# piljoong-jeong/nerf_meets_mlx

Measured on AMD Instinct MI355X. Metric: train+render rays/sec on Lego 800x800 (synthetic), coarse+fine 64+128, higher is better.
Workload: dtype split16 (fp16x2 render / bf16x2 train MFMA operands ~ 22 / 16 significand bits; fp32 accumulate)

## Files before the change

nerf_meets_mlx_amd/csrc/mlp.hip:

```cpp
#include "common.h"
#include "mlp_ring.h"
#include "mlp_layout.h"
#include "mlp_frag.h"
#include "mlp_arch2.h"
#include "hash_common.h"
#include "mlp_params.h"
#include "mlp_model.h"
#include "dw_split.h"
#include <limits.h>
#include <string.h>


namespace nerf {

extern int g_hash_combine_max_res;




constexpr int PACK_THREADS = (L::F_TOTAL + L::B_PADDED) * 64 + L::BI_TOTAL;
__device__ __forceinline__ void pack_part(int tid, const float* __restrict__ p, bf16x8* __restrict__ wf,
                                          bf16x8* __restrict__ wb, float* __restrict__ bias) {
  const int nf = L::F_TOTAL * 64, nb = L::B_PADDED * 64;
  if (tid < nf + nb) {
// ... 936 lines not shown
  for (int i = 0; i < DW_NPW; ++i) {
    const int nt = wr * DW_NPW + i;
    if (nt >= n_tiles) continue;
#pragma unroll
    for (int k = 0; k < 2; ++k) {
      const int kt = wc * 2 + k;
      if (kt >= k_tiles) continue;
      float* tile = slot + (8 * nt + kt) * 1024;
#pragma unroll
      for (int e = 0; e < 16; ++e) tile[((e & 3) + 8 * (e >> 2) + 4 * hh) * 32 + rr] = acc[i][k][e];
    }
    if (wc == 0 && jb.b_off >= 0) {
      const float tot = bsum[i] + __shfl_xor(bsum[i], 32, 64);
      if (hh == 0) slot[64 * 1024 + 32 * nt + rr] = tot;
    }
  }
}

__global__ void __launch_bounds__(256) mlp_dw_reduce_kernel(DwArgs a) {
  const int j = blockIdx.y;
  const DwJob jb = a.jobs[j];
  int first = 0;
  for (int q = 0; q < j; ++q) first += a.splits[q];
  const int S = a.splits[j];
  const int nw = jb.n_valid * jb.k_valid, nb = jb.b_off >= 0 ? jb.n_valid : 0;
  const float* base = a.partial + (size_t)first * DW_SLOT_FLOATS;
  for (int t = blockIdx.x * 256 + threadIdx.x; t < nw + nb; t += gridDim.x * 256) {
    const float* src;
    float* dst;
    if (t < nw) {
      const int n = t / jb.k_valid, k = t - n * jb.k_valid;
      src = base + (8 * (n >> 5) + (k >> 5)) * 1024 + (n & 31) * 32 + (k & 31);
      dst = a.grads + jb.w_off + (int64_t)n * jb.ldw + jb.col0 + k;
    } else {
      src = base + 64 * 1024 + (t - nw);
      dst = a.grads + jb.b_off + (t - nw);
    }
    float sum = 0.0f;
    int sidx = 0;
    for (; sidx + 8 <= S; sidx += 8) {
      float v[8];
#pragma unroll
      for (int q = 0; q < 8; ++q) v[q] = __builtin_nontemporal_load(src + (size_t)(sidx + q) * DW_SLOT_FLOATS);
#pragma unroll
      for (int q = 0; q < 8; ++q) sum += v[q];
    }
    for (; sidx < S; ++sidx) sum += __builtin_nontemporal_load(src + (size_t)sidx * DW_SLOT_FLOATS);
    *dst = sum;
  }
}



__global__ void __launch_bounds__(256) pack_img_kernel(const float* __restrict__ p, bf16x8* __restrict__ wf,
                                                       bf16x8* __restrict__ wb, float* __restrict__ bias, int out_ch) {
  const int tid = blockIdx.x * 256 + threadIdx.x;
  const int nf = LI::F_TOTAL * 64, nb = LI::B_PADDED * 64;
  if (tid < nf + nb) {
    const bool fw = tid < nf;
    const int t = fw ? tid : tid - nf;
    const int f = t >> 6, lane = t & 63, r = lane & 31, h = lane >> 5;
    bf16x8 v;
#pragma unroll
    for (int j = 0; j < 8; ++j)
      v[j] = (__bf16)(fw ? fwd_src_img(p, f, r, h, j, out_ch) : (f < LI::B_TOTAL ? bwd_src_img(p, f, r, h, j, out_ch) : 0.0f));
    (fw ? wf : wb)[t] = v;
  } else if (tid < nf + nb + LI::BI_TOTAL) {
    const int s = tid - nf - nb;
    bias[s] = s < 2048 ? p[LI::pb(s >> 8) + (s & 255)] : ((s - LI::BI_OUT) < out_ch ? p[LI::P_WO + out_ch * 256 + (s - LI::BI_OUT)] : 0.0f);
// ... 333 lines not shown
    {
      bf16x8 cat[ST][5];
#pragma unroll
      for (int k = 0; k < 4; ++k) cat[0][k] = zf[0][k];
      cat[0][4] = zal[0][0];
      layer_bwd<ST, 5, 2, true>(ws, LN::B_FA, cat, z1, mk[1], lane, ZSINK(LN::Z_L1));
    }
    layer_bwd<ST, 4, 2, true>(ws, LN::B_L1, z1, z0, mk[0], lane, ZSINK(LN::Z_L0));
#undef ZSINK
    if (a.d_x) {
      f32x16 acc;
#pragma unroll
      for (int i = 0; i < 16; ++i) acc[i] = 0.0f;
#pragma unroll
      for (int ns = 0; ns < 4; ++ns) acc = __builtin_amdgcn_mfma_f32_32x32x16_bf16(ws.frag(LN::B_L0 + ns, lane), z0[0][ns], acc, 0, 0, 0);
      if (m < a.M) {
#pragma unroll
        for (int q = 0; q < 4; ++q) {
          float4 o; o.x = acc[4 * q]; o.y = acc[4 * q + 1]; o.z = acc[4 * q + 2]; o.w = acc[4 * q + 3];
          *reinterpret_cast<float4*>(a.d_x + m * LN::CPOS + 8 * q + 4 * h) = o;
        }
      }
    }
  }
}

static int g_dw_wgs = 0;
static int g_dw_bias = -1;
static int g_bwd_stage = 0;
static int g_dw_ring_cap = 8;
static int g_dw_private = 4;
static int g_dw16_variant = 1;
static int g_dw_narrow_first = 1;
static int g_dw_job_mask = 0;
static int g_mlp_variant = 0;
static int g_ring_wgs = 0;
static int g_ngp_ray_major = 1;
int g_pass_queue = 1;
static int g_ring_split = 1;

static int cu_count() {
  constexpr int MAX_DEVICES = 64;
  static int n[MAX_DEVICES] = {};
  int dev = 0;
  if (hipGetDevice(&dev) != hipSuccess || dev < 0 || dev >= MAX_DEVICES) dev = 0;
  if (n[dev] == 0) {
    int v = 0;
    n[dev] = (hipDeviceGetAttribute(&v, hipDeviceAttributeMultiprocessorCount, dev) == hipSuccess && v > 0) ? v : 256;
  }
  return n[dev];
}
static inline int ring_wgs() { return g_ring_wgs > 0 ? g_ring_wgs : cu_count(); }
static inline unsigned ring_grid(int64_t ntiles) { return persistent_grid((ntiles + 7) / 8, ring_wgs()); }

struct Option { const char* key; int* var; bool (*rule)(int& v); const char* refusal; };
static bool opt_any(int&) { return true; }
static bool opt_flag(int& v) { v = v ? 1 : 0; return true; }
template <int LO, int HI> static bool opt_clamp(int& v) { v = v < LO ? LO : v > HI ? HI : v; return true; }
static const Option OPTIONS[] = {
    {"mlp_variant", &g_mlp_variant, opt_any, nullptr},
    {"ring_split", &g_ring_split, [](int& v) { return v == 1 || v == 2; }, "nerf_set_option: ring_split must be 1 or 2"},
    {"ring_workgroups", &g_ring_wgs, opt_clamp<0, INT_MAX>, nullptr},
    {"tile_pad16", &g_tile_pad16, opt_clamp<0, INT_MAX>, nullptr},
    {"dw_workgroups", &g_dw_wgs, opt_clamp<0, INT_MAX>, nullptr},
    {"dw_unit_bias", &g_dw_bias, opt_clamp<-1, INT_MAX>, nullptr},
    {"bwd_stage", &g_bwd_stage, opt_any, nullptr},
    {"dw_job_mask", &g_dw_job_mask, opt_any, nullptr},
    {"hash_combine_max_res", &g_hash_combine_max_res, opt_clamp<0, INT_MAX>, nullptr},
    {"ngp_ray_major", &g_ngp_ray_major, opt_flag, nullptr},
    {"dw22_variant", &s16::g_dw_variant, opt_flag, nullptr},
    {"dw16_variant", &g_dw16_variant, opt_clamp<0, 3>, nullptr},
    {"dw_private_tiles", &g_dw_private, opt_clamp<0, 4>, nullptr},
    {"dw_ring_cap", &g_dw_ring_cap, opt_clamp<2, 16>, nullptr},
    {"pass_queue", &g_pass_queue, opt_flag, nullptr},
    {"dw_narrow_first", &g_dw_narrow_first, opt_flag, nullptr},
    {"f22_tiles", &f22::g_tiles, [](int& v) { return v == 0 || v == 2 || v == 3; }, "nerf_set_option: f22_tiles must be 0 (automatic), 2 or 3"},
};

}

using namespace nerf;

extern "C" int nerf_set_option(const char* key, int value) {
  NERF_REQUIRE(key, NERF_E_NULL, "nerf_set_option: key is NULL");
  NERF_REQUIRE(strcmp(key, "mlp_precision") != 0, NERF_E_UNSUPPORTED,
               "nerf_set_option: \"mlp_precision\" is gone (ABI 3): set nerf_mlp_arch.precision of the model instead");
  for (const Option& o : OPTIONS) {
    if (strcmp(key, o.key)) continue;
    if (!o.rule(value)) return fail(NERF_E_UNSUPPORTED, "%s", o.refusal);
    *o.var = value;
    return NERF_OK;
  }
  return fail(NERF_E_UNSUPPORTED, "nerf_set_option: unknown key '%s'", key);
}

extern "C" int nerf_get_option(const char* key) {
  if (!key) return NERF_OPTION_UNKNOWN;
  for (const Option& o : OPTIONS)
    if (!strcmp(key, o.key)) return *o.var;
  return NERF_OPTION_UNKNOWN;
}

extern "C" int64_t nerf_mlp_param_count(const nerf_mlp_arch* arch) { return resolve(arch).params; }
extern "C" int64_t nerf_mlp_packed_bytes(const nerf_mlp_arch* arch) { return resolve(arch).packed_bytes; }
extern "C" int64_t nerf_mlp_acts_bytes(const nerf_mlp_arch* arch, int64_t M) { return resolve(arch).acts_bytes(M); }
extern "C" int64_t nerf_mlp_dz_bytes(const nerf_mlp_arch* arch, int64_t M) { return resolve(arch).dz_bytes(M); }

#define NERF_ARCH_MSG ": HIP kernels exist for (8x256, skip 4) with in=63+27 view head, or in=40 / no view head / out_ch<=4, and for (2x64, no skip) with in=32+16 view head"
// ... 130 lines not shown
}

static int view_forward(const Model& m, const void* packed, const float* x, const float* rays, const float* z, int64_t M, int n,
                        int freq_mode, float* out, void* acts, void* stream) {
  auto s = as_stream(stream);
  if (m.split() && !acts)
    return f22::forward(m.stream<void>(packed, S_F22), x, rays, z, M, n, freq_mode, out, ring_wgs(), s);
  if (m.split())
    return s16::forward(m.stream<void>(packed, S_S16), m.stream<float>(packed, S_BIAS), x, rays, z, M, n, freq_mode, out, acts,
                        m.astride(), ring_wgs(), s);
  if (m.prec == Prec::F32) return f32::forward(m.stream<void>(packed, S_F32), x, rays, z, M, n, freq_mode, out, acts, 0, s);
  return x ? launch_fwd<0>(m, packed, x, rays, z, M, n, freq_mode, out, acts, stream)
           : launch_fwd<1>(m, packed, x, rays, z, M, n, freq_mode, out, acts, stream);
}

extern "C" int nerf_mlp_forward(const nerf_mlp_arch* arch, const void* packed, const float* x, int64_t M, float* out,
                                void* stream) {
  return nerf_mlp_forward_train(arch, packed, x, M, out, nullptr, stream);
}

extern "C" int nerf_query_fused(const nerf_mlp_arch* arch, const void* packed, const float* rays, const float* z,
                                int64_t B, int n, int freq_mode, float* raw, void* acts, void* stream) {
  const Model m = resolve(arch);
  NERF_REQUIRE(m.ok && m.shape == Shape::View, NERF_E_UNSUPPORTED, "nerf_query_fused" NERF_ARCH_MSG);
  NERF_REQUIRE(n >= 1, NERF_E_SHAPE, "nerf_query_fused: n must be >= 1");
  if (B <= 0) return NERF_OK;
  NERF_REQUIRE(packed && rays && z && raw, NERF_E_NULL, "nerf_query_fused: NULL pointer");
  NERF_REQUIRE(freq_mode == 0 || freq_mode == 1, NERF_E_UNSUPPORTED, "nerf_query_fused: freq_mode must be 0 or 1");
  NERF_REQUIRE(B * (int64_t)n < (1ll << 31), NERF_E_SHAPE, "nerf_query_fused: B*n must be < 2^31 samples per call");
  return view_forward(m, packed, nullptr, rays, z, B * n, n, freq_mode, raw, acts, stream);
}

static int launch_dw_part(const Model& m, DwArgs& d, int nj, int64_t ntiles, const void* acts, void* dz, float* grads,
                          hipStream_t s, int kind, int slot_base, int max_wgs) {
  static_assert(DW_SPLIT_MAX_JOBS == DW_MAX_JOBS, "dw_split.h sizes its arrays for DwArgs::jobs");
  DwCost cost[DW_MAX_JOBS];
  for (int j = 0; j < nj; ++j) cost[j] = DwCost{d.jobs[j].nf, d.jobs[j].kf};
  int target_wgs = g_dw_wgs > 0 ? g_dw_wgs : cu_count();
  if (target_wgs > max_wgs) target_wgs = max_wgs;
  const int nw = dw_split(cost, nj, g_dw_bias >= 0 ? g_dw_bias : m.split() ? 2 : 128, target_wgs, (ntiles + 3) / 4, d.splits);
  NERF_REQUIRE(slot_base + nw <= DW_MAX_WGS, NERF_E_SHAPE, "nerf_mlp_backward: dw_workgroups must be <= %d", DW_MAX_WGS);
  bool all_tiny = true;
  for (int j = 0; j < nj; ++j) all_tiny = all_tiny && ((d.jobs[j].nf + 1) / 2) * ((d.jobs[j].kf + 1) / 2) <= 4;
  d.ntiles = (int)ntiles; d.astride = m.astride(); d.zstride = m.zstride();
  d.acts = acts; d.dz = dz; d.grads = grads;
  d.a_lo = m.info->a_lo; d.z_lo = m.info->z_lo; d.ring_cap = g_dw_ring_cap; d.private_max_tiles = g_dw_private;
  d.partial = m.dw_partial(dz, ntiles) + (size_t)slot_base * DW_SLOT_FLOATS;
  int rc;
  if (kind >= 2) {
    rc = launch_dw_wide_kernel(d, nw, kind == 2, s);
  } else if (kind == 1) {
    rc = s16::launch_dw_kernel(d, nw, true, s);
  } else if (g_dw16_variant == 3 || (g_dw16_variant == 1 && all_tiny)) {
    rc = s16::launch_dw_kernel(d, nw, false, s);
  } else {
    rc = launch<mlp_dw_kernel>("mlp dW", dim3(nw), dim3(64 * DW_WAVES), DW_LDS_BYTES, s, d);
  }
  if (rc) return rc;
  return launch<mlp_dw_reduce_kernel>("mlp dW reduce", dim3(257, nj), dim3(256), 0, s, d);
}

static int launch_dw(const Model& m, DwArgs& d, int nj, int64_t ntiles, const void* acts, void* dz, float* grads, hipStream_t s) {
  if (g_dw_job_mask) {
    hipError_t e = hipMemsetAsync(grads, 0, sizeof(float) * m.params, s);
    if (e != hipSuccess) return fail(NERF_E_HIP, "nerf_mlp_backward: memset: %s", hipGetErrorString(e));
  }
  const bool split_bf16 = m.split();
  if ((split_bf16 ? s16::g_dw_variant : g_dw16_variant) == 0)
    return launch_dw_part(m, d, nj, ntiles, acts, dz, grads, s, split_bf16 ? 1 : 0, 0, DW_MAX_WGS);
  DwArgs wide = d, rest = d;
  int nwide = 0, nrest = 0;
  for (int j = 0; j < nj; ++j) {
    if (d.jobs[j].nf == 16 && d.jobs[j].kf == 16) wide.jobs[nwide++] = d.jobs[j];
    else rest.jobs[nrest++] = d.jobs[j];
  }
  const int half = DW_MAX_WGS / 2;
  for (int turn = 0; turn < 2; ++turn) {
    const bool do_wide = (turn == 0) != (g_dw_narrow_first != 0);
    if (do_wide && nwide) {
      const int rc = launch_dw_part(m, wide, nwide, ntiles, acts, dz, grads, s, split_bf16 ? 2 : 3, half, half);
      if (rc) return rc;
    }
    if (!do_wide && nrest) {
      const int rc = launch_dw_part(m, rest, nrest, ntiles, acts, dz, grads, s, split_bf16 ? 1 : 0, 0, half);
      if (rc) return rc;
    }
  }
  return NERF_OK;
}

static int view_backward_chain(const Model& m, const void* packed, const void* acts, const float* d_raw, int64_t M, void* dz,
                               hipStream_t s) {
  const int64_t ntiles = (M + 31) / 32;
  if (m.split()) {
    if (g_bwd_stage != 2) {
      const int rcs = s16::backward_chain(m.stream<void>(packed, S_S16), acts, d_raw, M, dz, m.astride(), m.zstride(), ring_wgs(), s);
      if (rcs) return rcs;
    }
    return check_launch("mlp backward chain");
  }
  BwdArgs b;
  b.queue = nullptr;
  b.wb = m.stream<bf16x8>(packed, S_BWD);
  b.acts = acts; b.d_raw = d_raw; b.M = M; b.dz = dz; b.astride = m.astride(); b.zstride = m.zstride();
  const int variant = g_mlp_variant == 0 ? 3 : g_mlp_variant;
  const char* what = "mlp backward chain";
  if (variant >= 3) {
    b.queue = passq_slot();
    if (g_bwd_stage == 2) return check_launch(what);
    if (g_ring_split == 2)
      return launch<mlp_bwd_ring_kernel<SPLIT_NW, SPLIT_CHUNK>>(
          what, dim3(persistent_grid((ntiles + SPLIT_NW - 1) / SPLIT_NW, 2 * (int64_t)ring_wgs())), dim3(64 * SPLIT_NW), SPLIT_LDS_BYTES, s, b);
    return launch<mlp_bwd_ring_kernel<>>(what, dim3(ring_grid(ntiles)), dim3(512), RING_LDS_BYTES, s, b);
  }
  const int st = variant == 2 ? 2 : 1;
  const int64_t blocks = (ntiles + 4 * st - 1) / (4 * st);
  return with_bool(st == 1, [&](auto one) {
// ... 7 lines not shown
  NERF_REQUIRE(!d_x || m.shape == Shape::Small, NERF_E_UNSUPPORTED,
               "nerf_mlp_backward_inputs: input gradients exist for the (2x64) model only (the 8x256 models take fixed encodings)");
  NERF_REQUIRE(packed && acts && d_raw && dz && grads, NERF_E_NULL, "nerf_mlp_backward: NULL pointer");
  NERF_REQUIRE(M > 0, NERF_E_SHAPE, "nerf_mlp_backward: M must be > 0");
  auto s = as_stream(stream);
  const int64_t ntiles = (M + 31) / 32;
  if (m.prec == Prec::F32)
    return f32::backward(m.stream<void>(packed, S_F32), acts, d_raw, M, dz, grads, m.shape == Shape::Image ? m.out_ch : 0, s);
  int rc;
  if (m.shape == Shape::Small) {
    if (m.split()) {
      rc = s16x::small_backward_chain(m.stream<void>(packed, S_S16), acts, d_raw, M, dz, d_x, m.astride(), m.zstride(), s);
    } else {
      SmallArgs a;
      small_args(a, m, packed);
      a.d_raw = d_raw; a.acts = const_cast<void*>(acts); a.dz = dz; a.M = M; a.d_x = d_x;
      rc = launch<mlp_small_bwd_kernel>("mlp backward chain (2x64 model)", dim3(small_grid(ntiles)), dim3(512), LN::LDS_BYTES, s, a);
    }
  } else if (m.shape == Shape::Image) {
    if (m.split()) {
      rc = s16x::img_backward_chain(m.stream<void>(packed, S_S16), acts, d_raw, M, m.out_ch, dz, m.astride(), m.zstride(), ring_wgs(), s);
    } else {
      ImgArgs a;
      img_args(a, m, packed);
      a.d_out = d_raw; a.acts = const_cast<void*>(acts); a.dz = dz; a.M = M;
      rc = launch<mlp_img_bwd_ring_kernel>("mlp backward chain (image model)", dim3(ring_grid(ntiles)), dim3(512), RING_LDS_BYTES, s, a);
    }
  } else {
    rc = view_backward_chain(m, packed, acts, d_raw, M, dz, s);
    if (!rc && g_bwd_stage == 1) return NERF_OK;
  }
  if (rc) return rc;
  DwArgs d;
  const int nj = m.dw_jobs(d.jobs, m.shape == Shape::View ? g_dw_job_mask : 0);
  return launch_dw(m, d, nj, ntiles, acts, dz, grads, s);
}

static int ngp_query_fused_impl(const nerf_mlp_arch* arch, const void* packed, const float* rays, const float* z,
                                int64_t B, int n, const float* tables, const void* tables_half, int L, int log2_T, int F,
                                const int* resolutions_host, const float* lw_host, int sh_degree, float pos_scale,
                                float pos_offset, float* raw, void* acts, void* stream) {
  const Model m = resolve(arch);
  NERF_REQUIRE(m.ok && m.shape == Shape::Small, NERF_E_UNSUPPORTED, "nerf_ngp_query_fused: needs the (2x64, in 32+16) model");
  NERF_REQUIRE(L == 16 && F == 2 && sh_degree == 3, NERF_E_UNSUPPORTED,
               "nerf_ngp_query_fused: fused rows exist for 16 levels x 2 features + SH degree 3 (use nerf_ngp_encode + nerf_mlp_forward otherwise)");
  NERF_REQUIRE(log2_T >= 1 && log2_T <= 30, NERF_E_SHAPE, "nerf_ngp_query_fused: need 1<=log2_T<=30");
  if (B <= 0 || n <= 0) return NERF_OK;
  NERF_REQUIRE(packed && rays && z && tables && resolutions_host && raw, NERF_E_NULL, "nerf_ngp_query_fused: NULL pointer");
  const int64_t M = B * n;
  NERF_REQUIRE(M < (1ll << 31), NERF_E_SHAPE, "nerf_ngp_query_fused: B*n must be < 2^31");
  LevelTab lt;
  if (lw_host)
    NERF_REQUIRE(level_tab_fill(lt, lw_host, L), NERF_E_SHAPE, "nerf_ngp_query_fused_lw: level weights must be finite and in [0, 1]");
  if (m.split()) {
    s16x::SmallQuery q;
    q.rays = rays; q.z = z; q.n = n; q.tables = tables; q.T = 1u << log2_T; q.pos_scale = pos_scale; q.pos_offset = pos_offset;
    for (int l = 0; l < 32; ++l) q.res[l] = l < L ? (float)resolutions_host[l] : 0.0f;
    q.B = B; q.ray_major = g_ngp_ray_major;
    q.use_lw = lw_host != nullptr;
    if (lw_host) for (int l = 0; l < 32; ++l) q.lw[l] = lt.w[l];
    return s16x::small_forward(m.stream<void>(packed, S_S16), m.stream<float>(packed, S_BIAS), nullptr, M, raw, acts, m.astride(), &q,
                               as_stream(stream));
  }
  SmallArgs a;
  small_args(a, m, packed);
  a.out = raw; a.acts = acts; a.M = M; a.rays = rays; a.z = z; a.n = n; a.tables = tables; a.T = 1u << log2_T;
  a.tables_h = static_cast<const uint32_t*>(tables_half);
  a.pos_scale = pos_scale; a.pos_offset = pos_offset;
// ... 98 lines not shown
```

nerf_meets_mlx_amd/csrc/mlp_frag.h:

```cpp
#pragma once
#include "mlp_layout.h"

namespace nerf {

struct Chan { int kind, dim, band; };
__host__ __device__ constexpr Chan chan_of(int c, int limit) {
  if (c < 3) return Chan{0, c, 0};
  if (c >= limit) return Chan{3, 0, 0};
  return Chan{((c - 3) % 6) >= 3 ? 2 : 1, (c - 3) % 3, (c - 3) / 6};
}

__device__ inline float fwd_src(const float* __restrict__ p, int f, int r, int h, int j) {
  int nt, ks;
  if (f < L::F_L1) {
    nt = f / 4; ks = f % 4;
    const int kk = kperm(ks, h, j);
    return kk < 63 ? p[L::P_W0 + (32 * nt + r) * 63 + kk] : 0.0f;
  }
  if (f < L::F_L5) {
    const int l = 1 + (f - L::F_L1) / 128, g = (f - L::F_L1) % 128;
    nt = g / 16; ks = g % 16;
    return p[L::pw(l) + (32 * nt + r) * 256 + kperm(ks, h, j)];
  }
  if (f < L::F_L6) {
    const int g = f - L::F_L5;
    nt = g / 20; ks = g % 20;
    const int kk = kperm(ks, h, j), n = 32 * nt + r;
    if (kk < 64) return kk < 63 ? p[L::P_W5 + n * 319 + kk] : 0.0f;
    return p[L::P_W5 + n * 319 + 63 + (kk - 64)];
  }
  if (f < L::F_FA) {
    const int l = 6 + (f - L::F_L6) / 128, g = (f - L::F_L6) % 128;
    nt = g / 16; ks = g % 16;
    return p[L::pw(l) + (32 * nt + r) * 256 + kperm(ks, h, j)];
  }
  if (f < L::F_DIR) {
    const int g = f - L::F_FA;
    nt = g / 16; ks = g % 16;
    const int kk = kperm(ks, h, j);
    if (nt < 8) return p[L::P_WF + (32 * nt + r) * 256 + kk];
    return r == 0 ? p[L::P_WA + kk] : 0.0f;
  }
  if (f < L::F_RGB) {
    const int g = f - L::F_DIR;
    nt = g / 18; ks = g % 18;
    const int kk = kperm(ks, h, j), n = 32 * nt + r;
    if (kk < 256) return p[L::P_WD + n * 283 + kk];
    return (kk - 256) < 27 ? p[L::P_WD + n * 283 + kk] : 0.0f;
  }
  ks = f - L::F_RGB;
  return r < 3 ? p[L::P_WR + r * 128 + kperm(ks, h, j)] : 0.0f;
}

__device__ inline float bwd_src(const float* __restrict__ p, int f, int r, int h, int j) {
  if (f < L::B_DIR) {
    const int nn = kperm(0, h, j);
    return nn < 3 ? p[L::P_WR + nn * 128 + 32 * f + r] : 0.0f;
  }
  if (f < L::B_FA) {
    const int g = f - L::B_DIR, kt = g / 8, ns = g % 8;
    return p[L::P_WD + kperm(ns, h, j) * 283 + 32 * kt + r];
  }
  if (f < L::B_L7) {
    const int g = f - L::B_FA, kt = g / 17, ns = g % 17;
    const int nn = kperm(ns, h, j);
    if (ns < 16) return p[L::P_WF + nn * 256 + 32 * kt + r];
    return nn == 256 ? p[L::P_WA + 32 * kt + r] : 0.0f;
  }
  const int g = f - L::B_L7, li = g / 128, q = g % 128, kt = q / 16, ns = q % 16;
  const int l = 7 - li, nn = kperm(ns, h, j), row = 32 * kt + r;
  if (l == 5) return p[L::P_W5 + nn * 319 + 63 + row];
  return p[L::pw(l) + nn * 256 + row];
}

__device__ __forceinline__ bf16x8* frag_ptr(void* base, int64_t tile, int64_t stride16, int slot, int r, int h) {
  char* tb = reinterpret_cast<char*>(base) + tile * stride16 * 16;
  return reinterpret_cast<bf16x8*>(tb + slot * 1024 + (unsigned)(32 * r + 16 * h));
}

#ifndef NERF_NT_STORES
#define NERF_NT_STORES 1
#endif
constexpr bool g_nt_stores = NERF_NT_STORES != 0;

__device__ __forceinline__ void store_frag(void* base, int64_t tile, int64_t stride16, int slot, const bf16x8& v,
                                           int r, int h) {
#if NERF_ABLATE == 7
  asm volatile("" :: "v"(v));
  return;
#endif
#if NERF_ABLATE == 8
  tile = tile & 7;
#endif
  if (g_nt_stores) __builtin_nontemporal_store(v, frag_ptr(base, tile, stride16, slot, r, h));
  else *frag_ptr(base, tile, stride16, slot, r, h) = v;
}
template <int COUNT>
__device__ __forceinline__ void store_frags(void* base, int64_t tile, int64_t stride16, int slot0,
                                            const bf16x8 (&frags)[COUNT], int r, int h) {
#pragma unroll
  for (int k = 0; k < COUNT; ++k) store_frag(base, tile, stride16, slot0 + k, frags[k], r, h);
}
struct NoSink {
  __device__ __forceinline__ void put(int, int, const bf16x8&) const {}
};
// ... 60 lines not shown
}
template <int B>
__device__ __forceinline__ bf16x2 keep_where(bf16x2 p, unsigned w) {
  unsigned sel, r;
  asm("v_pk_lshrrev_b16 %0, %2, %1 op_sel_hi:[0,1]" : "=v"(sel) : "v"(w), "n"(B));
  sel &= 0x00010001u;
  asm("v_pk_mul_lo_u16 %0, %1, %2" : "=v"(r) : "v"(__builtin_bit_cast(unsigned, p)), "v"(sel));
  return __builtin_bit_cast(bf16x2, r);
}

template <bool RELU, bool MASKOUT>
__device__ __forceinline__ void finish_quarter(const f32x16& acc, int q, int nt, bf16x8& lo, bf16x8& hi, u32x4& mask) {
  unsigned w = 0;
#pragma unroll
  for (int p = 0; p < 2; ++p) {
    const int i = 4 * q + 2 * p, k = 2 * q + p;
    const bf16x2 pr = RELU ? relu_pack(acc[i], acc[i + 1]) : pack2(acc[i], acc[i + 1]);
    if (MASKOUT) w |= nonzero_bits(pr) << k;
    if (i < 8) { lo[i] = pr[0]; lo[i + 1] = pr[1]; } else { hi[i - 8] = pr[0]; hi[i - 7] = pr[1]; }
  }
  if (MASKOUT) mask[nt >> 1] |= w << (8 * (nt & 1));
}

__host__ __device__ constexpr int quarter_pos(int ks_count, int q) {
  return ks_count >= 8 ? (q * ks_count) / 4 + 1 : (q < ks_count ? q : ks_count - 1);
}

struct DwJob {
  int dz_slot, nf;
  int act_slot, kf;
  int w_off, ldw, col0;
  int n_valid, k_valid;
  int b_off;
};
constexpr int DW_MAX_JOBS = 16;
struct DwArgs {
  DwJob jobs[DW_MAX_JOBS];
  int splits[DW_MAX_JOBS];
  int ntiles;
  int64_t astride, zstride;
  const void* acts;
  const void* dz;
  float* grads;
  float* partial;
  int ring_cap;
  int private_max_tiles;
  int a_lo, z_lo;
};
constexpr int DW_SLOT_FLOATS = 64 * 1024 + 256;
constexpr int DW_MAX_WGS = 512;
constexpr int64_t DW_PARTIAL_BYTES = (int64_t)DW_MAX_WGS * DW_SLOT_FLOATS * 4;
int launch_dw_wide_kernel(const DwArgs& d, int workgroups, bool split_bf16, hipStream_t s);

}
```

nerf_meets_mlx_amd/csrc/mlp_layout.h:

```cpp
#pragma once
#include "mlp_ring.h"
#include "mlp_params.h"

namespace nerf {

namespace L {

constexpr int F_L0 = 0, F_L1 = 32, F_L5 = 544, F_L6 = 704, F_L7 = 832, F_FA = 960, F_DIR = 1104, F_RGB = 1176;
constexpr int F_TOTAL = 1184;
constexpr int B_RGB = 0, B_DIR = 4, B_FA = 68, B_L7 = 204, B_L6 = 332, B_L5 = 460, B_L4 = 588;
constexpr int B_TOTAL = 1100, B_PADDED = 1120;
constexpr int BI_FEAT = 2048, BI_ALPHA = 2304, BI_DIR = 2336, BI_RGB = 2464, BI_TOTAL = 2496;
constexpr int F16_TOTAL = 1172, F16_PADDED = 1184;
constexpr int64_t F16_OFFSET = (int64_t)(F_TOTAL + B_PADDED) * 1024 + BI_TOTAL * 4;
constexpr int64_t PACKED_BYTES = F16_OFFSET + (int64_t)F16_PADDED * 1024;

constexpr int A_PE = 0, A_DPE = 4, A_H0 = 6;
constexpr int A_FEAT = 134, A_HD = 150;
constexpr int A_MASK = 158, A_SLOTS = 167;
constexpr int Z_L0 = 0;
constexpr int Z_F = 128, Z_A = 144, Z_D = 145, Z_RGB = 153, Z_SLOTS = 154;
}

__host__ __device__ constexpr int kperm(int ks, int h, int j) { return 16 * ks + 8 * (j >> 2) + 4 * h + (j & 3); }

namespace L16 {
constexpr int F_L0 = 0, F_L1 = 32, F_L5 = 544, F_L6 = 704, F_L7 = 832, F_FA = 960, F_DIR = 1096, F_RGB = 1168;
constexpr int CHUNKS = L::F16_PADDED / RING_CHUNK;
}
__host__ __device__ constexpr int kperm16(int ks, int g, int j) { return 32 * ks + 16 * (j >> 2) + 4 * g + (j & 3); }
__host__ __device__ constexpr int pos_chan16(int ks, int g, int j) {
  const int sl = 8 * ks + j;
  if (sl < 12) return 3 + 6 * (2 * g + sl / 6) + (sl % 6);
  if (sl < 15) return 3 + 6 * (8 + (g >> 1)) + 3 * (g & 1) + (sl - 12);
  return g < 3 ? g : -1;
}
__host__ __device__ constexpr int dir_chan16(int g, int j) {
  if (j < 6) return 3 + 6 * g + j;
  return (j == 6 && g < 3) ? g : -1;
}

__device__ inline float fwd_src16(const float* __restrict__ p, int f, int i, int g, int j) {
  if (f < L16::F_L1) {
    const int nt = f / 2, ch = pos_chan16(f % 2, g, j);
    return ch >= 0 ? p[L::P_W0 + (16 * nt + i) * 63 + ch] : 0.0f;
  }
  if (f < L16::F_L5) {
    const int q = f - L16::F_L1, l = 1 + q / 128, r = q % 128;
    return p[L::pw(l) + (16 * (r / 8) + i) * 256 + kperm16(r % 8, g, j)];
  }
  if (f < L16::F_L6) {
    const int q = f - L16::F_L5, n = 16 * (q / 10) + i, ks = q % 10;
    if (ks < 2) { const int ch = pos_chan16(ks, g, j); return ch >= 0 ? p[L::P_W5 + n * 319 + ch] : 0.0f; }
    return p[L::P_W5 + n * 319 + 63 + kperm16(ks - 2, g, j)];
  }
  if (f < L16::F_FA) {
    const int q = f - L16::F_L6, l = 6 + q / 128, r = q % 128;
// ... 20 lines not shown
```

nerf_meets_mlx_amd/csrc/mlp_model.h:

```cpp
#pragma once
#include "mlp_arch2.h"
#include "mlp_frag.h"
#include "mlp32.h"
#include "mlp22.h"
#include "mlp_s16.h"
#include "mlp_s16x.h"

namespace nerf {

inline int g_tile_pad16 = 0;

enum class Shape { View, Image, Small };
enum class Prec { Bf16, F32, Split };
enum Stream { S_FWD, S_BWD, S_BIAS, S_FWD16, S_F32, S_F22, S_S16, S_COUNT };

struct DebugSlot { int slot, nfrag; };
#define NERF_HIDDEN8(b) {b, 16}, {b + 16, 16}, {b + 32, 16}, {b + 48, 16}, {b + 64, 16}, {b + 80, 16}, {b + 96, 16}, {b + 112, 16}

constexpr DwJob view_pos(int l) { return {L::Z_L0 + 16 * l, 16, L::A_H0 + 16 * (l - 1), 16, L::pw(l), 256, 0, 256, 256, L::pb(l)}; }
constexpr DwJob img_pos(int l) { return {LI::Z_L0 + 16 * l, 16, LI::A_H0 + 16 * (l - 1), 16, LI::pw(l), 256, 0, 256, 256, LI::pb(l)}; }
constexpr DwJob VIEW_JOBS[] = {
    {L::Z_L0, 16, L::A_PE, 4, L::P_W0, 63, 0, 256, 63, L::P_B0},
    view_pos(1), view_pos(2), view_pos(3), view_pos(4),
    {L::Z_L0 + 80, 16, L::A_H0 + 64, 16, L::P_W5, 319, 63, 256, 256, L::P_B5},
    {L::Z_L0 + 80, 16, L::A_PE, 4, L::P_W5, 319, 0, 256, 63, -1},
    view_pos(6), view_pos(7),
    {L::Z_F, 16, L::A_H0 + 112, 16, L::P_WF, 256, 0, 256, 256, L::P_BF},
    {L::Z_A, 1, L::A_H0 + 112, 16, L::P_WA, 256, 0, 1, 256, L::P_BA},
    {L::Z_D, 8, L::A_FEAT, 16, L::P_WD, 283, 0, 128, 256, L::P_BD},
    {L::Z_D, 8, L::A_DPE, 2, L::P_WD, 283, 256, 128, 27, -1},
    {L::Z_RGB, 1, L::A_HD, 8, L::P_WR, 128, 0, 3, 128, L::P_BR},
};
constexpr DwJob IMG_JOBS[] = {
    {LI::Z_L0, 16, LI::A_X, 3, LI::P_W0, 40, 0, 256, 40, LI::P_B0},
    img_pos(1), img_pos(2), img_pos(3), img_pos(4),
    {LI::Z_L0 + 80, 16, LI::A_H0 + 64, 16, LI::P_W5, 296, 40, 256, 256, LI::P_B5},
    {LI::Z_L0 + 80, 16, LI::A_X, 3, LI::P_W5, 296, 0, 256, 40, -1},
    img_pos(6), img_pos(7),
    {LI::Z_OUT, 1, LI::A_H0 + 112, 16, LI::P_WO, 256, 0, 0, 256, 0},
};
constexpr DwJob SMALL_JOBS[] = {
    {LN::Z_L0, 4, LN::A_X, 2, LN::P_W0, 32, 0, 64, 32, LN::P_B0},
    {LN::Z_L1, 4, LN::A_H0, 4, LN::P_W1, 64, 0, 64, 64, LN::P_B1},
    {LN::Z_F, 4, LN::A_H1, 4, LN::P_WF, 64, 0, 64, 64, LN::P_BF},
    {LN::Z_A, 1, LN::A_H1, 4, LN::P_WA, 64, 0, 1, 64, LN::P_BA},
    {LN::Z_D, 2, LN::A_FEAT, 4, LN::P_WD, 80, 0, 32, 64, LN::P_BD},
    {LN::Z_D, 2, LN::A_DX, 1, LN::P_WD, 80, 64, 32, 16, -1},
    {LN::Z_RGB, 1, LN::A_HD, 2, LN::P_WR, 32, 0, 3, 32, LN::P_BR},
};

struct ShapeInfo {
  int64_t params;
  int f_frags, b_frags, bias_floats;
  int f16_frags;
  int64_t split_bytes;
  int a_slots[2], z_slots[2];
  int a_lo, z_lo;
  const DwJob* jobs; int njobs;
  DebugSlot debug[2][12];
};
constexpr ShapeInfo SHAPES[3] = {
    {L::P_TOTAL, L::F_TOTAL, L::B_PADDED, L::BI_TOTAL, L::F16_PADDED, s16::PACKED_BYTES,
     {L::A_SLOTS, s16::A_SLOTS}, {L::Z_SLOTS, s16::Z_SLOTS}, s16::A_LO, s16::Z_LO, VIEW_JOBS, sizeof(VIEW_JOBS) / sizeof(DwJob),
     {{NERF_HIDDEN8(L::A_H0), {L::A_FEAT, 16}, {L::A_HD, 8}, {L::A_PE, 4}, {L::A_DPE, 2}},
      {NERF_HIDDEN8(L::Z_L0), {L::Z_F, 16}, {L::Z_D, 8}, {L::Z_A, 1}, {L::Z_RGB, 1}}}},
    {LI::P_WO, LI::F_TOTAL, LI::B_PADDED, LI::BI_TOTAL, 0, s16x::IMG_PACKED_BYTES,
     {LI::A_SLOTS, s16x::IMG_A_SLOTS}, {LI::Z_SLOTS, s16x::IMG_Z_SLOTS}, s16x::IMG_A_LO, s16x::IMG_Z_LO, IMG_JOBS, sizeof(IMG_JOBS) / sizeof(DwJob),
     {{NERF_HIDDEN8(LI::A_H0), {0, 0}, {0, 0}, {LI::A_X, 3}, {0, 0}},
      {NERF_HIDDEN8(LI::Z_L0), {LI::Z_OUT, 1}, {0, 0}, {0, 0}, {0, 0}}}},
    {LN::P_TOTAL, LN::F_PADDED, LN::B_PADDED, LN::BI_TOTAL, 0, s16x::SM_PACKED_BYTES,
     {LN::A_SLOTS, s16x::SM_A_SLOTS}, {LN::Z_SLOTS, s16x::SM_Z_SLOTS}, s16x::SM_A_LO, s16x::SM_Z_LO, SMALL_JOBS, sizeof(SMALL_JOBS) / sizeof(DwJob),
     {{{LN::A_H0, 4}, {LN::A_H1, 4}, {0, 0}, {0, 0}, {0, 0}, {0, 0}, {0, 0}, {0, 0}, {LN::A_FEAT, 4}, {LN::A_HD, 2}, {LN::A_X, 2}, {LN::A_DX, 1}},
      {{LN::Z_L0, 4}, {LN::Z_L1, 4}, {0, 0}, {0, 0}, {0, 0}, {0, 0}, {0, 0}, {0, 0}, {LN::Z_F, 4}, {LN::Z_D, 2}, {LN::Z_A, 1}, {LN::Z_RGB, 1}}}},
};
#undef NERF_HIDDEN8

inline int64_t padded_tiles(int64_t M) { return (((M + 31) / 32) + 7) / 8 * 8; }

struct Model {
  bool ok = false;
  Shape shape; Prec prec; int out_ch;
  const ShapeInfo* info;
  int64_t params, packed_bytes;
  int64_t off[S_COUNT];
  int a_slots, z_slots;

  bool split() const { return prec == Prec::Split; }
  template <class T> const T* stream(const void* packed, Stream s) const { return reinterpret_cast<const T*>(static_cast<const char*>(packed) + off[s]); }
  template <class T> T* stream(void* packed, Stream s) const { return reinterpret_cast<T*>(static_cast<char*>(packed) + off[s]); }
  int64_t astride() const { return (int64_t)a_slots * 64 + g_tile_pad16; }
  int64_t zstride() const { return (int64_t)z_slots * 64 + g_tile_pad16; }
  int64_t acts_bytes(int64_t M) const { return !ok || M < 0 ? -1 : prec == Prec::F32 ? f32::acts_bytes(M) : padded_tiles(M) * astride() * 16; }
  int64_t dz_bytes(int64_t M) const {
    return !ok || M < 0 ? -1 : prec == Prec::F32 ? f32::dz_bytes(M) : padded_tiles(M) * zstride() * 16 + DW_PARTIAL_BYTES;
  }
  float* dw_partial(void* dz, int64_t ntiles) const { return reinterpret_cast<float*>(static_cast<char*>(dz) + padded_tiles(ntiles * 32) * zstride() * 16); }
  int dw_jobs(DwJob* dst, int mask) const {
    int nj = 0;
    for (int j = 0; j < info->njobs; ++j) {
      if (mask && !((mask >> j) & 1)) continue;
      dst[nj] = info->jobs[j];
      if (shape == Shape::Image && j == info->njobs - 1) { dst[nj].n_valid = out_ch; dst[nj].b_off = LI::P_WO + out_ch * 256; }
      ++nj;
    }
    return nj;
  }
  DebugSlot debug_slot(int kind, int layer) const {
    return (layer < 0 || layer > 11 || (kind != 0 && kind != 1)) ? DebugSlot{0, 0} : info->debug[kind][layer];
  }
};

inline Model resolve(const nerf_mlp_arch* a) {
  Model m{};
  m.params = m.packed_bytes = -1;
  if (!a) return m;
  if (a->precision != 0 && a->precision != 16 && a->precision != 32 && a->precision != 22) return m;
  m.prec = a->precision == 32 ? Prec::F32 : a->precision == 22 ? Prec::Split : Prec::Bf16;
  if (m.prec == Prec::F32 && !(a->n_layers == 8 && a->width == 256)) return m;
  if (a->n_layers == 2 && a->width == 64 && a->skip_layer < 0 && a->use_viewdirs == 1 && a->in_pos == 32 && a->in_dir == 16) m.shape = Shape::Small;
  else if (a->n_layers != 8 || a->width != 256 || a->skip_layer != 4) return m;
  else if (a->use_viewdirs == 1 && a->in_pos == 63 && a->in_dir == 27) m.shape = Shape::View;
  else if (a->use_viewdirs == 0 && a->in_pos == 40 && a->out_ch >= 1 && a->out_ch <= 4) m.shape = Shape::Image;
  else return m;
  const ShapeInfo& s = SHAPES[(int)m.shape];
  m.info = &s;
  m.out_ch = a->out_ch;
  m.params = s.params + (m.shape == Shape::Image ? (int64_t)a->out_ch * 257 : 0);
  m.a_slots = s.a_slots[m.split()]; m.z_slots = s.z_slots[m.split()];
  for (int i = 0; i < S_COUNT; ++i) m.off[i] = -1;
  int64_t end = 0;
  auto put = [&](Stream st, int64_t bytes) { m.off[st] = end; end += bytes; };
// ... 14 lines not shown
```

Before: 1.224 million.

## Factor feature/dir0 weight gradients through a shared dZ_alpha+dZ_D job and post-kernel

Adds a factored dW path for the split-precision view model. The separate feature-layer and dir0 weight-gradient jobs are replaced by one job that computes alpha plus an auxiliary 128x256 product G and the dir bias sum into a spare partial slot. A new post kernel then recovers W_feature, b_feature, W_dir0 and b_dir gradients by chaining through the packed forward weights in double precision. The aim is to cut the MFMA reduction work over all samples, at the cost of an extra launch and a change in rounding because the packed bf16 hi/lo weights are used.

```diff
diff --git a/nerf_meets_mlx_amd/csrc/mlp.hip b/nerf_meets_mlx_amd/csrc/mlp.hip
--- a/nerf_meets_mlx_amd/csrc/mlp.hip
+++ b/nerf_meets_mlx_amd/csrc/mlp.hip
@@ -992,9 +992,18 @@
       const int n = t / jb.k_valid, k = t - n * jb.k_valid;
       src = base + (8 * (n >> 5) + (k >> 5)) * 1024 + (n & 31) * 32 + (k & 31);
       dst = a.grads + jb.w_off + (int64_t)n * jb.ldw + jb.col0 + k;
+      if (jb.aux_row0 > 0) {
+        if (n >= jb.aux_row0) dst = a.aux + (n - jb.aux_row0) * jb.k_valid + k;
+        else if (n >= jb.n_grad) continue;
+      }
     } else {
-      src = base + 64 * 1024 + (t - nw);
-      dst = a.grads + jb.b_off + (t - nw);
+      const int n = t - nw;
+      src = base + 64 * 1024 + n;
+      dst = a.grads + jb.b_off + n;
+      if (jb.aux_row0 > 0) {
+        if (n >= jb.aux_row0) dst = a.aux + (jb.n_valid - jb.aux_row0) * jb.k_valid + (n - jb.aux_row0);
+        else if (n >= jb.n_grad) continue;
+      }
     }
     float sum = 0.0f;
     int sidx = 0;
@@ -1394,6 +1403,7 @@
 static int g_dw_private = 4;
 static int g_dw16_variant = 1;
 static int g_dw_narrow_first = 1;
+static int g_dw_factor = 1;
 static int g_dw_job_mask = 0;
 static int g_mlp_variant = 0;
 static int g_ring_wgs = 0;
@@ -1436,6 +1446,7 @@
     {"dw_ring_cap", &g_dw_ring_cap, opt_clamp<2, 16>, nullptr},
     {"pass_queue", &g_pass_queue, opt_flag, nullptr},
     {"dw_narrow_first", &g_dw_narrow_first, opt_flag, nullptr},
+    {"dw_factor", &g_dw_factor, opt_flag, nullptr},
     {"f22_tiles", &f22::g_tiles, [](int& v) { return v == 0 || v == 2 || v == 3; }, "nerf_set_option: f22_tiles must be 0 (automatic), 2 or 3"},
 };
 
@@ -1632,10 +1643,11 @@
 }
 
 static int launch_dw_part(const Model& m, DwArgs& d, int nj, int64_t ntiles, const void* acts, void* dz, float* grads,
-                          hipStream_t s, int kind, int slot_base, int max_wgs) {
+                          hipStream_t s, int kind, int slot_base, int max_wgs, int aux_slot = -1) {
   static_assert(DW_SPLIT_MAX_JOBS == DW_MAX_JOBS, "dw_split.h sizes its arrays for DwArgs::jobs");
   DwCost cost[DW_MAX_JOBS];
-  for (int j = 0; j < nj; ++j) cost[j] = DwCost{d.jobs[j].nf, d.jobs[j].kf};
+  constexpr int SHARED_JOB_EXTRA_UNITS = 12;
+  for (int j = 0; j < nj; ++j) cost[j] = DwCost{d.jobs[j].nf, d.jobs[j].kf + (d.jobs[j].aux_row0 > 0 ? SHARED_JOB_EXTRA_UNITS : 0)};
   int target_wgs = g_dw_wgs > 0 ? g_dw_wgs : cu_count();
   if (target_wgs > max_wgs) target_wgs = max_wgs;
   const int nw = dw_split(cost, nj, g_dw_bias >= 0 ? g_dw_bias : m.split() ? 2 : 128, target_wgs, (ntiles + 3) / 4, d.splits);
@@ -1646,6 +1658,7 @@
   d.acts = acts; d.dz = dz; d.grads = grads;
   d.a_lo = m.info->a_lo; d.z_lo = m.info->z_lo; d.ring_cap = g_dw_ring_cap; d.private_max_tiles = g_dw_private;
   d.partial = m.dw_partial(dz, ntiles) + (size_t)slot_base * DW_SLOT_FLOATS;
+  d.aux = aux_slot >= 0 ? m.dw_partial(dz, ntiles) + (size_t)aux_slot * DW_SLOT_FLOATS : nullptr;
   int rc;
   if (kind >= 2) {
     rc = launch_dw_wide_kernel(d, nw, kind == 2, s);
@@ -1660,7 +1673,8 @@
   return launch<mlp_dw_reduce_kernel>("mlp dW reduce", dim3(257, nj), dim3(256), 0, s, d);
 }
 
-static int launch_dw(const Model& m, DwArgs& d, int nj, int64_t ntiles, const void* acts, void* dz, float* grads, hipStream_t s) {
+static int launch_dw(const Model& m, const void* packed, DwArgs& d, int nj, int64_t ntiles, const void* acts, void* dz, float* grads,
+                     hipStream_t s, bool factored) {
   if (g_dw_job_mask) {
     hipError_t e = hipMemsetAsync(grads, 0, sizeof(float) * m.params, s);
     if (e != hipSuccess) return fail(NERF_E_HIP, "nerf_mlp_backward: memset: %s", hipGetErrorString(e));
@@ -1682,7 +1696,9 @@
       if (rc) return rc;
     }
     if (!do_wide && nrest) {
-      const int rc = launch_dw_part(m, rest, nrest, ntiles, acts, dz, grads, s, split_bf16 ? 1 : 0, 0, half);
+      int rc = launch_dw_part(m, rest, nrest, ntiles, acts, dz, grads, s, split_bf16 ? 1 : 0, 0, half, factored ? half : -1);
+      if (!rc && factored)
+        rc = launch_dw_factor_post(m.stream<void>(packed, S_S16), m.stream<float>(packed, S_BIAS), rest.aux, grads, s);
       if (rc) return rc;
     }
   }
@@ -1756,8 +1772,10 @@
   }
   if (rc) return rc;
   DwArgs d;
-  const int nj = m.dw_jobs(d.jobs, m.shape == Shape::View ? g_dw_job_mask : 0);
-  return launch_dw(m, d, nj, ntiles, acts, dz, grads, s);
+  const int mask = m.shape == Shape::View ? g_dw_job_mask : 0;
+  const bool factored = g_dw_factor && m.can_factor() && !mask && s16::g_dw_variant != 0;
+  const int nj = m.dw_jobs(d.jobs, mask, factored);
+  return launch_dw(m, packed, d, nj, ntiles, acts, dz, grads, s, factored);
 }
 
 static int ngp_query_fused_impl(const nerf_mlp_arch* arch, const void* packed, const float* rays, const float* z,
diff --git a/nerf_meets_mlx_amd/csrc/mlp_dwf.hip b/nerf_meets_mlx_amd/csrc/mlp_dwf.hip
--- /dev/null
+++ b/nerf_meets_mlx_amd/csrc/mlp_dwf.hip
@@ -0,0 +1,81 @@
+#include "common.h"
+#include "launch.h"
+#include "mlp_frag.h"
+
+namespace nerf {
+
+constexpr int DWF_ROWS = 2;
+constexpr int DWF_BLOCKS_F = 256 / DWF_ROWS, DWF_BLOCKS_D = 128 / DWF_ROWS;
+
+__device__ __forceinline__ double pair_value(const __bf16* __restrict__ wf, const FragElem& e) {
+  FragElem hi = e, lo = e;
+  hi.f = 2 * e.f; lo.f = 2 * e.f + 1;
+  return (double)(float)wf[frag_elem_offset(hi)] + (double)(float)wf[frag_elem_offset(lo)];
+}
+
+__global__ void __launch_bounds__(256) mlp_dw_factor_post_kernel(const __bf16* __restrict__ wf, const float* __restrict__ bias,
+                                                                 const float* __restrict__ aux, float* __restrict__ grads) {
+  __shared__ double sh[256 * DWF_ROWS];
+  __shared__ double sdb[128];
+  const int t = threadIdx.x;
+  const float* G = aux + DWF_G;
+  const float* dbD = aux + DWF_DB;
+  double acc[DWF_ROWS];
+#pragma unroll
+  for (int q = 0; q < DWF_ROWS; ++q) acc[q] = 0.0;
+  if (blockIdx.x < DWF_BLOCKS_F) {
+    const int k0 = DWF_ROWS * blockIdx.x;
+    for (int e = t; e < 128 * DWF_ROWS; e += 256) {
+      const int j = e / DWF_ROWS, q = e % DWF_ROWS;
+      sh[e] = pair_value(wf, fwd_elem_dir0(j, k0 + q));
+    }
+    if (t < 128) sdb[t] = (double)dbD[t];
+    __syncthreads();
+    for (int j = 0; j < 128; ++j) {
+      const double g = (double)G[j * 256 + t];
+#pragma unroll
+      for (int q = 0; q < DWF_ROWS; ++q) acc[q] = __builtin_fma(sh[j * DWF_ROWS + q], g, acc[q]);
+    }
+#pragma unroll
+    for (int q = 0; q < DWF_ROWS; ++q) grads[L::P_WF + (k0 + q) * 256 + t] = (float)acc[q];
+    if (t < DWF_ROWS) {
+      double b = 0.0;
+      for (int j = 0; j < 128; ++j) b = __builtin_fma(sh[j * DWF_ROWS + t], sdb[j], b);
+      grads[L::P_BF + k0 + t] = (float)b;
+    }
+  } else {
+    const int j0 = DWF_ROWS * (blockIdx.x - DWF_BLOCKS_F);
+    for (int e = t; e < 256 * DWF_ROWS; e += 256) {
+      const int q = e / 256, i = e % 256;
+      sh[i * DWF_ROWS + q] = (double)G[(j0 + q) * 256 + i];
+    }
+    __syncthreads();
+    for (int ks = 0; ks < 16; ++ks) {
+      for (int h = 0; h < 2; ++h) {
+        const FragElem e0 = fwd_elem_feature(t, kperm(ks, h, 0));
+        FragElem eh = e0, el = e0;
+        eh.f = 2 * e0.f; el.f = 2 * e0.f + 1;
+        const bf16x8 vh = *reinterpret_cast<const bf16x8*>(wf + frag_elem_offset(eh));
+        const bf16x8 vl = *reinterpret_cast<const bf16x8*>(wf + frag_elem_offset(el));
+#pragma unroll
+        for (int jj = 0; jj < 8; ++jj) {
+          const double w = (double)(float)vh[jj] + (double)(float)vl[jj];
+          const int i = kperm(ks, h, jj);
+#pragma unroll
+          for (int q = 0; q < DWF_ROWS; ++q) acc[q] = __builtin_fma(w, sh[i * DWF_ROWS + q], acc[q]);
+        }
+      }
+    }
+    const double bf = (double)bias[L::BI_FEAT + t];
+#pragma unroll
+    for (int q = 0; q < DWF_ROWS; ++q) grads[L::P_WD + (j0 + q) * 283 + t] = (float)__builtin_fma(bf, (double)dbD[j0 + q], acc[q]);
+    if (t < DWF_ROWS) grads[L::P_BD + j0 + t] = dbD[j0 + t];
+  }
+}
+
+int launch_dw_factor_post(const void* packed_s16, const float* bias_slots, const float* aux, float* grads, hipStream_t s) {
+  return launch<mlp_dw_factor_post_kernel>("mlp dW post step (factored feature / dir0)", dim3(DWF_BLOCKS_F + DWF_BLOCKS_D), dim3(256), 0, s,
+                                           static_cast<const __bf16*>(packed_s16), bias_slots, aux, grads);
+}
+
+}
diff --git a/nerf_meets_mlx_amd/csrc/mlp_frag.h b/nerf_meets_mlx_amd/csrc/mlp_frag.h
--- a/nerf_meets_mlx_amd/csrc/mlp_frag.h
+++ b/nerf_meets_mlx_amd/csrc/mlp_frag.h
@@ -11,66 +11,12 @@
 }
 
 __device__ inline float fwd_src(const float* __restrict__ p, int f, int r, int h, int j) {
-  int nt, ks;
-  if (f < L::F_L1) {
-    nt = f / 4; ks = f % 4;
-    const int kk = kperm(ks, h, j);
-    return kk < 63 ? p[L::P_W0 + (32 * nt + r) * 63 + kk] : 0.0f;
-  }
-  if (f < L::F_L5) {
-    const int l = 1 + (f - L::F_L1) / 128, g = (f - L::F_L1) % 128;
-    nt = g / 16; ks = g % 16;
-    return p[L::pw(l) + (32 * nt + r) * 256 + kperm(ks, h, j)];
-  }
-  if (f < L::F_L6) {
-    const int g = f - L::F_L5;
-    nt = g / 20; ks = g % 20;
-    const int kk = kperm(ks, h, j), n = 32 * nt + r;
-    if (kk < 64) return kk < 63 ? p[L::P_W5 + n * 319 + kk] : 0.0f;
-    return p[L::P_W5 + n * 319 + 63 + (kk - 64)];
-  }
-  if (f < L::F_FA) {
-    const int l = 6 + (f - L::F_L6) / 128, g = (f - L::F_L6) % 128;
-    nt = g / 16; ks = g % 16;
-    return p[L::pw(l) + (32 * nt + r) * 256 + kperm(ks, h, j)];
-  }
-  if (f < L::F_DIR) {
-    const int g = f - L::F_FA;
-    nt = g / 16; ks = g % 16;
-    const int kk = kperm(ks, h, j);
-    if (nt < 8) return p[L::P_WF + (32 * nt + r) * 256 + kk];
-    return r == 0 ? p[L::P_WA + kk] : 0.0f;
-  }
-  if (f < L::F_RGB) {
-    const int g = f - L::F_DIR;
-    nt = g / 18; ks = g % 18;
-    const int kk = kperm(ks, h, j), n = 32 * nt + r;
-    if (kk < 256) return p[L::P_WD + n * 283 + kk];
-    return (kk - 256) < 27 ? p[L::P_WD + n * 283 + kk] : 0.0f;
-  }
-  ks = f - L::F_RGB;
-  return r < 3 ? p[L::P_WR + r * 128 + kperm(ks, h, j)] : 0.0f;
+  const int i = fwd_index(f, r, h, j);
+  return i >= 0 ? p[i] : 0.0f;
 }
-
 __device__ inline float bwd_src(const float* __restrict__ p, int f, int r, int h, int j) {
-  if (f < L::B_DIR) {
-    const int nn = kperm(0, h, j);
-    return nn < 3 ? p[L::P_WR + nn * 128 + 32 * f + r] : 0.0f;
-  }
-  if (f < L::B_FA) {
-    const int g = f - L::B_DIR, kt = g / 8, ns = g % 8;
-    return p[L::P_WD + kperm(ns, h, j) * 283 + 32 * kt + r];
-  }
-  if (f < L::B_L7) {
-    const int g = f - L::B_FA, kt = g / 17, ns = g % 17;
-    const int nn = kperm(ns, h, j);
-    if (ns < 16) return p[L::P_WF + nn * 256 + 32 * kt + r];
-    return nn == 256 ? p[L::P_WA + 32 * kt + r] : 0.0f;
-  }
-  const int g = f - L::B_L7, li = g / 128, q = g % 128, kt = q / 16, ns = q % 16;
-  const int l = 7 - li, nn = kperm(ns, h, j), row = 32 * kt + r;
-  if (l == 5) return p[L::P_W5 + nn * 319 + 63 + row];
-  return p[L::pw(l) + nn * 256 + row];
+  const int i = bwd_index(f, r, h, j);
+  return i >= 0 ? p[i] : 0.0f;
 }
 
 __device__ __forceinline__ bf16x8* frag_ptr(void* base, int64_t tile, int64_t stride16, int slot, int r, int h) {
@@ -197,6 +143,7 @@
   int w_off, ldw, col0;
   int n_valid, k_valid;
   int b_off;
+  int n_grad, aux_row0;
 };
 constexpr int DW_MAX_JOBS = 16;
 struct DwArgs {
@@ -211,10 +158,14 @@
   int ring_cap;
   int private_max_tiles;
   int a_lo, z_lo;
+  float* aux;
 };
 constexpr int DW_SLOT_FLOATS = 64 * 1024 + 256;
 constexpr int DW_MAX_WGS = 512;
 constexpr int64_t DW_PARTIAL_BYTES = (int64_t)DW_MAX_WGS * DW_SLOT_FLOATS * 4;
+constexpr int DWF_G = 0, DWF_DB = 128 * 256, DWF_FLOATS = DWF_DB + 128;
+static_assert(DWF_FLOATS <= DW_SLOT_FLOATS, "the factored job's result fits one partial-tile slot");
+int launch_dw_factor_post(const void* packed_s16, const float* bias_slots, const float* aux, float* grads, hipStream_t s);
 int launch_dw_wide_kernel(const DwArgs& d, int workgroups, bool split_bf16, hipStream_t s);
 
 }
diff --git a/nerf_meets_mlx_amd/csrc/mlp_index.h b/nerf_meets_mlx_amd/csrc/mlp_index.h
--- /dev/null
+++ b/nerf_meets_mlx_amd/csrc/mlp_index.h
@@ -0,0 +1,93 @@
+#pragma once
+#if !defined(__HIPCC__) && !defined(__host__)
+#define __host__
+#define __device__
+#endif
+#include "mlp_params.h"
+
+namespace nerf {
+
+namespace L {
+constexpr int F_L0 = 0, F_L1 = 32, F_L5 = 544, F_L6 = 704, F_L7 = 832, F_FA = 960, F_DIR = 1104, F_RGB = 1176;
+constexpr int F_TOTAL = 1184;
+constexpr int B_RGB = 0, B_DIR = 4, B_FA = 68, B_L7 = 204, B_L6 = 332, B_L5 = 460, B_L4 = 588;
+constexpr int B_TOTAL = 1100, B_PADDED = 1120;
+}
+
+__host__ __device__ constexpr int kperm(int ks, int h, int j) { return 16 * ks + 8 * (j >> 2) + 4 * h + (j & 3); }
+__host__ __device__ constexpr int kperm_ks(int kk) { return kk >> 4; }
+__host__ __device__ constexpr int kperm_h(int kk) { return (kk >> 2) & 1; }
+__host__ __device__ constexpr int kperm_j(int kk) { return 4 * ((kk >> 3) & 1) + (kk & 3); }
+
+__host__ __device__ constexpr int fwd_index(int f, int r, int h, int j) {
+  if (f < L::F_L1) {
+    const int nt = f / 4, ks = f % 4;
+    const int kk = kperm(ks, h, j);
+    return kk < 63 ? L::P_W0 + (32 * nt + r) * 63 + kk : -1;
+  }
+  if (f < L::F_L5) {
+    const int l = 1 + (f - L::F_L1) / 128, g = (f - L::F_L1) % 128;
+    const int nt = g / 16, ks = g % 16;
+    return L::pw(l) + (32 * nt + r) * 256 + kperm(ks, h, j);
+  }
+  if (f < L::F_L6) {
+    const int g = f - L::F_L5;
+    const int nt = g / 20, ks = g % 20;
+    const int kk = kperm(ks, h, j), n = 32 * nt + r;
+    if (kk < 64) return kk < 63 ? L::P_W5 + n * 319 + kk : -1;
+    return L::P_W5 + n * 319 + 63 + (kk - 64);
+  }
+  if (f < L::F_FA) {
+    const int l = 6 + (f - L::F_L6) / 128, g = (f - L::F_L6) % 128;
+    const int nt = g / 16, ks = g % 16;
+    return L::pw(l) + (32 * nt + r) * 256 + kperm(ks, h, j);
+  }
+  if (f < L::F_DIR) {
+    const int g = f - L::F_FA;
+    const int nt = g / 16, ks = g % 16;
+    const int kk = kperm(ks, h, j);
+    if (nt < 8) return L::P_WF + (32 * nt + r) * 256 + kk;
+    return r == 0 ? L::P_WA + kk : -1;
+  }
+  if (f < L::F_RGB) {
+    const int g = f - L::F_DIR;
+    const int nt = g / 18, ks = g % 18;
+    const int kk = kperm(ks, h, j), n = 32 * nt + r;
+    if (kk < 256) return L::P_WD + n * 283 + kk;
+    return (kk - 256) < 27 ? L::P_WD + n * 283 + kk : -1;
+  }
+  const int ks = f - L::F_RGB;
+  return r < 3 ? L::P_WR + r * 128 + kperm(ks, h, j) : -1;
+}
+
+__host__ __device__ constexpr int bwd_index(int f, int r, int h, int j) {
+  if (f < L::B_DIR) {
+    const int nn = kperm(0, h, j);
+    return nn < 3 ? L::P_WR + nn * 128 + 32 * f + r : -1;
+  }
+  if (f < L::B_FA) {
+    const int g = f - L::B_DIR, kt = g / 8, ns = g % 8;
+    return L::P_WD + kperm(ns, h, j) * 283 + 32 * kt + r;
+  }
+  if (f < L::B_L7) {
+    const int g = f - L::B_FA, kt = g / 17, ns = g % 17;
+    const int nn = kperm(ns, h, j);
+    if (ns < 16) return L::P_WF + nn * 256 + 32 * kt + r;
+    return nn == 256 ? L::P_WA + 32 * kt + r : -1;
+  }
+  const int g = f - L::B_L7, li = g / 128, q = g % 128, kt = q / 16, ns = q % 16;
+  const int l = 7 - li, nn = kperm(ns, h, j), row = 32 * kt + r;
+  if (l == 5) return L::P_W5 + nn * 319 + 63 + row;
+  return L::pw(l) + nn * 256 + row;
+}
+
+struct FragElem { int f, r, h, j; };
+__host__ __device__ constexpr FragElem fwd_elem_feature(int row, int col) {
+  return FragElem{L::F_FA + 16 * (row >> 5) + kperm_ks(col), row & 31, kperm_h(col), kperm_j(col)};
+}
+__host__ __device__ constexpr FragElem fwd_elem_dir0(int row, int col) {
+  return FragElem{L::F_DIR + 18 * (row >> 5) + kperm_ks(col), row & 31, kperm_h(col), kperm_j(col)};
+}
+__host__ __device__ constexpr int frag_elem_offset(const FragElem& e) { return (e.f * 64 + 32 * e.h + e.r) * 8 + e.j; }
+
+}
diff --git a/nerf_meets_mlx_amd/csrc/mlp_layout.h b/nerf_meets_mlx_amd/csrc/mlp_layout.h
--- a/nerf_meets_mlx_amd/csrc/mlp_layout.h
+++ b/nerf_meets_mlx_amd/csrc/mlp_layout.h
@@ -1,15 +1,12 @@
 #pragma once
 #include "mlp_ring.h"
 #include "mlp_params.h"
+#include "mlp_index.h"
 
 namespace nerf {
 
 namespace L {
 
-constexpr int F_L0 = 0, F_L1 = 32, F_L5 = 544, F_L6 = 704, F_L7 = 832, F_FA = 960, F_DIR = 1104, F_RGB = 1176;
-constexpr int F_TOTAL = 1184;
-constexpr int B_RGB = 0, B_DIR = 4, B_FA = 68, B_L7 = 204, B_L6 = 332, B_L5 = 460, B_L4 = 588;
-constexpr int B_TOTAL = 1100, B_PADDED = 1120;
 constexpr int BI_FEAT = 2048, BI_ALPHA = 2304, BI_DIR = 2336, BI_RGB = 2464, BI_TOTAL = 2496;
 constexpr int F16_TOTAL = 1172, F16_PADDED = 1184;
 constexpr int64_t F16_OFFSET = (int64_t)(F_TOTAL + B_PADDED) * 1024 + BI_TOTAL * 4;
@@ -22,7 +19,6 @@
 constexpr int Z_F = 128, Z_A = 144, Z_D = 145, Z_RGB = 153, Z_SLOTS = 154;
 }
 
-__host__ __device__ constexpr int kperm(int ks, int h, int j) { return 16 * ks + 8 * (j >> 2) + 4 * h + (j & 3); }
 
 namespace L16 {
 constexpr int F_L0 = 0, F_L1 = 32, F_L5 = 544, F_L6 = 704, F_L7 = 832, F_FA = 960, F_DIR = 1096, F_RGB = 1168;
diff --git a/nerf_meets_mlx_amd/csrc/mlp_model.h b/nerf_meets_mlx_amd/csrc/mlp_model.h
--- a/nerf_meets_mlx_amd/csrc/mlp_model.h
+++ b/nerf_meets_mlx_amd/csrc/mlp_model.h
@@ -30,6 +30,12 @@
     {L::Z_D, 8, L::A_FEAT, 16, L::P_WD, 283, 0, 128, 256, L::P_BD},
     {L::Z_D, 8, L::A_DPE, 2, L::P_WD, 283, 256, 128, 27, -1},
     {L::Z_RGB, 1, L::A_HD, 8, L::P_WR, 128, 0, 3, 128, L::P_BR},
+};
+static_assert(L::Z_D == L::Z_A + 1, "d alpha and dZ_D are adjacent dZ fragments");
+constexpr DwJob VIEW_JOBS_FACTORED[] = {
+    VIEW_JOBS[0], VIEW_JOBS[1], VIEW_JOBS[2], VIEW_JOBS[3], VIEW_JOBS[4], VIEW_JOBS[5], VIEW_JOBS[6], VIEW_JOBS[7], VIEW_JOBS[8],
+    {L::Z_A, 9, L::A_H0 + 112, 16, L::P_WA, 256, 0, 16 + 128, 256, L::P_BA, 1, 16},
+    VIEW_JOBS[12], VIEW_JOBS[13],
 };
 constexpr DwJob IMG_JOBS[] = {
     {LI::Z_L0, 16, LI::A_X, 3, LI::P_W0, 40, 0, 256, 40, LI::P_B0},
@@ -95,8 +101,13 @@
     return !ok || M < 0 ? -1 : prec == Prec::F32 ? f32::dz_bytes(M) : padded_tiles(M) * zstride() * 16 + DW_PARTIAL_BYTES;
   }
   float* dw_partial(void* dz, int64_t ntiles) const { return reinterpret_cast<float*>(static_cast<char*>(dz) + padded_tiles(ntiles * 32) * zstride() * 16); }
-  int dw_jobs(DwJob* dst, int mask) const {
+  bool can_factor() const { return shape == Shape::View && prec == Prec::Split; }
+  int dw_jobs(DwJob* dst, int mask, bool factored = false) const {
     int nj = 0;
+    if (factored && can_factor() && !mask) {
+      for (const DwJob& j : VIEW_JOBS_FACTORED) dst[nj++] = j;
+      return nj;
+    }
     for (int j = 0; j < info->njobs; ++j) {
       if (mask && !((mask >> j) & 1)) continue;
       dst[nj] = info->jobs[j];
```

New measurement: 1.243 million, median of 6. 1.5% higher.
